# xiaochuanle/MECAT

Measured on AMD Instinct MI355X. Metric: candidate overlaps/sec, higher is better.
Workload: dtype int32

## Files before the change

mecat_amd/csrc/dw_extend2.hip:

```cpp
#include <stdio.h>
#include <stdlib.h>
#include <string.h>

#include <algorithm>
#include <type_traits>

#include "cns_fwd.h"
#include "dw_defs.h"
#include "dw_helpers.h"

#ifndef RCAP
#define RCAP 1024
#endif
#define SEQ_WORDS2 48
constexpr int FULL_BAND_TOL = (int)(0.3 * SEG_BLK), FULL_MAX_D = (int)(.3 * (SEG_BLK + SEG_BLK));
struct StagedLds {
    uint32_t Qp[SEQ_WORDS2][AL_WAVES * 2];
    uint32_t Tp[SEQ_WORDS2][AL_WAVES * 2];
};
#define STAGED_T_BYTES ((int)offsetof(StagedLds, Tp))
typedef __attribute__((address_space(3))) uint16_t lds_u16_t;
typedef __attribute__((address_space(3))) int16_t lds_i16_t;
__device__ __forceinline__ int ring_ld(uint32_t base, uint32_t pos) { return (int)*(lds_i16_t*)(uintptr_t)(base | (pos & (2 * RCAP - 2))); }
__device__ __forceinline__ void ring_st(uint32_t base, uint32_t pos, int x) { *(lds_u16_t*)(uintptr_t)(base | (pos & (2 * RCAP - 2))) = (uint16_t)x; }

__device__ __forceinline__ int sep_word(int rec) { return rec ^ (int)0xE000FFFFu; }

#define BALLOT(p) __builtin_amdgcn_ballot_w64(p)

template <int CTRL> __device__ __forceinline__ int dpp_max_step(int v) {
    return max(v, __builtin_amdgcn_update_dpp((int)0x80000000, v, CTRL, 0xf, 0xf, false));
}
__device__ __forceinline__ int half_max(int v0) {
    int v;
    asm("s_nop 1\n\tv_max_i32_dpp %0, %1, %1 quad_perm:[1,0,3,2] row_mask:0xf bank_mask:0xf" : "=v"(v) : "v"(v0));
    v = dpp_max_step<0x4E>(v);
    v = dpp_max_step<0x141>(v);
    v = dpp_max_step<0x140>(v);
    int r = v, w = v;
    asm("s_nop 1\n\tv_permlane16_swap_b32 %0, %1\n\ts_nop 1" : "+v"(r), "+v"(w));
    return max(r, w);
}
__device__ __forceinline__ int half_min(int v) { return -half_max(-v); }

template <int OFF> __device__ __forceinline__ unsigned long long bits_at(int n) {
    unsigned long long r;
    asm("s_bfm_b64 %0, %1, %2" : "=s"(r) : "s"(n), "n"(OFF));
    return r;
}

typedef uint32_t dw_u32x2 __attribute__((ext_vector_type(2)));
__device__ __forceinline__ unsigned long long pair64(uint32_t lo, uint32_t hi) {
    const dw_u32x2 v = {lo, hi};
    return __builtin_bit_cast(unsigned long long, v);
}
__device__ __forceinline__ uint32_t word_lo(unsigned long long v) { return __builtin_bit_cast(dw_u32x2, v).x; }
__device__ __forceinline__ uint32_t word_hi(unsigned long long v) { return __builtin_bit_cast(dw_u32x2, v).y; }

__device__ __forceinline__ unsigned long long pass_bits(int n) {
    unsigned long long r;
    asm("s_bfm_b64 %0, %1, 0" : "=s"(r) : "s"(n));
    return r;
}

template <int OFF> __device__ __forceinline__ unsigned long long clamped_bits_at(int n) {
    unsigned long long r;
    int c;
    asm("s_min_i32 %1, %2, 32\n\ts_max_i32 %1, %1, 0\n\ts_bfm_b64 %0, %1, %3" : "=s"(r), "=&s"(c) : "s"(n), "n"(OFF) : "scc");
    return r;
}

#define ROWS_ENDED 0xc0000000u
__device__ __forceinline__ unsigned long long snake_step_end(unsigned long long at_lim, unsigned long long amask, int nn,
                                                             unsigned long long& ended, int& rows_more) {
    unsigned long long more;
    int mark;
    asm("s_and_b64 %[more], %[at], %[am]\n\t"
        "s_cbranch_scc0 1f\n\t"
        "v_cmp_eq_u32 vcc, 32, %[nn]\n\t"
        "s_and_b64 vcc, vcc, %[more]\n\t"
        "s_cselect_b64 %[more], 0, %[more]\n\t"
        "s_cselect_b32 %[mark], 0, 0xc0000000\n\t"
        "s_or_b32 %[rm], %[rm], %[mark]\n\t"
        "s_or_b64 %[en], %[en], %[more]\n\t"
        "s_mov_b64 %[more], vcc\n"
        "1:"
        : [more] "=&s"(more), [mark] "=&s"(mark), [en] "+s"(ended), [rm] "+s"(rows_more)
        : [at] "s"(at_lim), [am] "s"(amask), [nn] "v"(nn)
        : "vcc", "scc");
    return more;
}
__device__ __forceinline__ int rows_more_value(int rows_more, bool marked) {
    return marked ? (int)(((unsigned)rows_more + 1u) & ~ROWS_ENDED) - 1 : rows_more;
}

#ifndef DW2_WAVES_PER_SIMD
#define DW2_WAVES_PER_SIMD 8
#endif
#ifndef CNS_FWD_WAVES_PER_SIMD
#define CNS_FWD_WAVES_PER_SIMD 8
#endif
template <bool CNS>
__global__ __launch_bounds__(AL_BLOCK, CNS ? CNS_FWD_WAVES_PER_SIMD : DW2_WAVES_PER_SIMD) void dw_extend2(const uint32_t* __restrict__ rpac, const mhip_offset_t* __restrict__ roffs,
                                                       const uint32_t* __restrict__ qpac, const mhip_offset_t* __restrict__ qoffs,
                                                       const mhip_aln_job* __restrict__ jobs, int n, DirResult* __restrict__ dres,
                                                       DwHandover* __restrict__ hand, unsigned int* __restrict__ hand_count,
                                                       unsigned int* __restrict__ cursor, unsigned long long* __restrict__ counters,
                                                       const CnsFwdArgs ca) {
    struct DwLds {
        uint16_t rings[AL_WAVES * 2][RCAP];
        StagedLds staged;
    };
    static_assert(offsetof(DwLds, staged) % 2048 == 0 && 32 * SEQ_WORDS2 <= 2048 && sizeof(uint32_t) * AL_WAVES * 2 == 32,
                  "a window's byte offset x2 & ~31 and the address of a half's word 0 have no bit in common");
    __shared__ __attribute__((aligned(2 * RCAP))) DwLds lds;
    const int lane = lane_id(), hh = lane >> 5, sl = lane & 31;
    const int half_u = (threadIdx.x >> 6) * 2 + hh;
    const uint32_t rbase = (uint32_t)(uintptr_t)(lds_u16_t*)&lds.rings[half_u][0];
    const uint32_t ubase = (uint32_t)(uintptr_t)(lds_u32_t*)&lds.staged.Qp[0][half_u];
    unsigned int cells = 0, nblocks = 0, nhand = 0;
#ifdef MECAT_DW_STATS
    unsigned long long nrows = 0, nidle = 0, nwide = 0;
    unsigned long long tk_rows = 0, tk_setup = 0, tk_ended = 0, tk_trace = 0, tk_acct = 0, n_outer = 0, n_setup = 0, n_ended = 0, n_pass3 = 0;
    unsigned long long nh[8] = {0, 0, 0, 0, 0, 0, 0, 0};
    unsigned long long q16[6] = {0, 0, 0, 0, 0, 0};
    unsigned long long snake2 = 0;
    unsigned long long n_one = 0, n_one32 = 0;
    const unsigned long long tk_start = wall_clock64();
#define DWS_T(var) const unsigned long long var = wall_clock64()
#define DWS_ADD(acc, a, b) acc += (b) - (a)
#else
#define DWS_T(var)
#define DWS_ADD(acc, a, b)
#endif

    bool need_unit = true, exhausted = false;
    bool setup = true;
    bool inblock = false;
    unsigned int unit = 0;
    SeqView q, t;
    q.pac = qpac; t.pac = rpac; q.off = 0; t.off = 0; q.A = q.B = t.A = t.B = 0; q.comp = t.comp = 0;
    int query_size = 0, target_size = 0, qidx = 0, tidx = 0;
    int Rq = 0, Rt = 0, Rm = 0, Rc = 0, Rb = 0;
    int q_len2 = 0, t_len2 = 0, last_block = 0, band_tol2 = 0, max_d = 0;
    int best_m = -1, mk_l = 0, nslot = 0, aligned = 0, end_x = 0, end_k = 0, end_d = 0, end_mk = 0, d = 0;
    int sepv = sep_word(1);
    int cut = 0;
    unsigned int lin_l = 0;
    unsigned int pb_l = 0;
    unsigned int rlin_l = 0;
    int dlim = 0;
    unsigned int logpos = 0, logend = 0, blk_log0 = 0, blkpos = 0, blkend = 0;
    bool cns_bad = false;
    unsigned long long fl0 = 0, fl1 = 0, fl2 = 0;
    int last_ns = 0;

    while (true) {
#ifdef MECAT_DW_STATS
        n_outer += 1;
        n_setup += BALLOT(setup) ? 1u : 0u;
#endif
        DWS_T(t_a);
        if (BALLOT(setup)) {
            if (setup && need_unit) {
                unsigned int u = 0;
                if (sl == 0) u = atomicAdd(cursor, 1u);
                u = __shfl(u, hh << 5);
                if (u >= 2u * (unsigned)n) { exhausted = true; setup = false; mk_l = 4 * sl; nslot = 0; dlim = 0; }
                else {
                    unit = u;
                    const mhip_aln_job jb = jobs[u >> 1];
                    const int right = u & 1;
                    const int qsize = qoffs[jb.qid_local].size, tsize = roffs[jb.sid_local].size;
                    q.off = qoffs[jb.qid_local].offset; q.comp = jb.chain;
                    t.off = roffs[jb.sid_local].offset; t.comp = 0;
                    const int qs0 = right ? jb.qstart : jb.qstart - 1, step = right ? 1 : -1;
                    if (jb.chain) { q.A = qsize - 1 - qs0; q.B = -step; } else { q.A = qs0; q.B = step; }
                    t.A = right ? jb.sstart : jb.sstart - 1; t.B = step;
                    if (right) { query_size = qsize - jb.qstart; target_size = tsize - jb.sstart; }
                    else { query_size = jb.qstart; target_size = jb.sstart; }
                    if (jb.qstart < 0 || jb.sstart < 0) { query_size = 0; target_size = 0; }
                    qidx = tidx = 0;
                    Rq = Rt = Rm = Rc = Rb = 0;
                    need_unit = false;
                    if (CNS) { logpos = ca.logbase[u]; logend = ca.logbase[u + 1]; blkpos = ca.blockbase[u]; blkend = ca.blockbase[u + 1]; cns_bad = false; }
                }
            }
            if (setup) {
                const int qleft = query_size - qidx, tleft = target_size - tidx;
                int qblk, tblk, band_tol;
                if (CNS) {
                    const int ext = min(qleft, tleft);
                    if (ext > SEG_BLK + 100) { qblk = SEG_BLK; last_block = 0; } else { qblk = max(ext, 0); last_block = 1; }
                    tblk = qblk;
                    if (last_block) {
                        band_tol = (int)(0.3 * qblk);
                        max_d = (int)(2.0 * ca.error_rate * (qblk + qblk));
                    } else { band_tol = FULL_BAND_TOL; max_d = ca.full_max_d; }
                    blk_log0 = logpos;
                    if (logend - logpos < (unsigned)max_d) { cns_bad = true; max_d = 0; }
                } else {
                if (qleft < SEG_BLK + 100 || tleft < SEG_BLK + 100) {
                    qblk = min(qleft, (int)(tleft + tleft * 0.2));
                    tblk = min(tleft, (int)(qleft + qleft * 0.2));
                    last_block = 1;
                    qblk = max(qblk, 0);
                    tblk = max(tblk, 0);
                    band_tol = (int)(0.3 * (qblk > tblk ? qblk : tblk));
                    max_d = (int)(.3 * (qblk + tblk));
                } else { qblk = SEG_BLK; tblk = SEG_BLK; last_block = 0; band_tol = FULL_BAND_TOL; max_d = FULL_MAX_D; }
                }
                static_assert((SEG_BLK + 99) * 6 / 5 <= 16 * (SEQ_WORDS2 - 1), "the longest block and one 16-base window fit the staged words");
                const int trips = BALLOT(max(qblk, tblk) > 512) ? 2 : 1;
#pragma unroll 1
                for (int w = sl, i = 0; i < trips; w += 32, ++i) {
                    lds_u32_t* const sw = (lds_u32_t*)(uintptr_t)(ubase + 32u * (unsigned)w);
                    if (w * 16 < qblk) sw[0] = view_word_le(q, qidx + w * 16);
                    if (w * 16 < tblk) sw[STAGED_T_BYTES / 4] = view_word_le(t, tidx + w * 16);
                }
                if (sl < 3) ring_st(rbase, 2u * sl, sl == 1 ? 0 : -2);
                best_m = -2; mk_l = 4 * sl; nslot = 1; sepv = sep_word(1); cut = 0;
                aligned = 0; end_x = 0; end_k = 0; end_d = 0; d = 0;
                lin_l = 6u + 2u * sl; pb_l = 2u * sl; rlin_l = 2u * sl;
                dlim = max_d; inblock = true;
                q_len2 = 2 * qblk; t_len2 = 2 * tblk; band_tol2 = 2 * band_tol;
                setup = false;
            }
            __builtin_amdgcn_wave_barrier();
        }
        if (!BALLOT(!exhausted)) break;
        const int k_offset = max_d;
        DWS_T(t_b);
        DWS_ADD(tk_setup, t_a, t_b);

        const unsigned long long inmask = BALLOT(inblock);
        bool row_ok;
        unsigned long long ended = 0;
        int NJ = 1;
        auto band_update = [&](const int NJ, const int m0, const int mp, auto both_tag, int& sa, int& sb) __attribute__((always_inline)) {
            constexpr bool BOTH = decltype(both_tag)::value;
            int first, last;
            int pk = 0;
            if (NJ == 1) {
                const unsigned long long q0 = BALLOT(m0 >= best_m - band_tol2);
                if (BOTH) {
                    const unsigned int wa = (unsigned int)q0, wb = (unsigned int)(q0 >> 32);
                    const int fa = __builtin_ctz(wa), fb = __builtin_ctz(wb);
                    sa = 33 - (fa + __builtin_clz(wa));
                    sb = 33 - (fb + __builtin_clz(wb));
                    unsigned long long pkw = (unsigned int)(sa | (fa << 8)) | ((unsigned long long)(unsigned int)(sb | (fb << 8)) << 32);
                    asm("" : "+s"(pkw));
                    pk = (int)(unsigned int)(pkw >> (hh << 5));
                    first = pk >> 8;
                    last = first + (pk & 0xff) - 2;
                } else {
                    const unsigned int m32 = (unsigned int)(q0 >> (hh << 5));
                    int lz;
                    asm("v_ffbl_b32 %0, %1" : "=v"(first) : "v"(m32));
                    asm("v_ffbh_u32 %0, %1" : "=v"(lz) : "v"(m32));
                    last = 31 - lz;
                }
            } else if (NJ == 2) {
                const int thr = best_m - band_tol2;
                const unsigned long long q0 = BALLOT(mp >= thr), q1 = BALLOT(m0 >= thr);
                if (BOTH) {
                    const unsigned long long wa = pair64(word_lo(q0), word_lo(q1)), wb = pair64(word_hi(q0), word_hi(q1));
                    const int fa = __builtin_ctzll(wa), fb = __builtin_ctzll(wb);
                    sa = 65 - (fa + __builtin_clzll(wa));
                    sb = 65 - (fb + __builtin_clzll(wb));
                    unsigned long long pkw = (unsigned int)(sa | (fa << 8)) | ((unsigned long long)(unsigned int)(sb | (fb << 8)) << 32);
                    asm("" : "+s"(pkw));
                    pk = (int)(unsigned int)(pkw >> (hh << 5));
                    first = pk >> 8;
                    last = first + (pk & 0xff) - 2;
                } else {
                    const unsigned int lo32 = (unsigned int)(q0 >> (hh << 5)), hi32 = (unsigned int)(q1 >> (hh << 5));
                    unsigned int fl, fh, ll, lh;
                    asm("v_ffbl_b32 %0, %1" : "=v"(fl) : "v"(lo32));
                    asm("v_ffbl_b32 %0, %1" : "=v"(fh) : "v"(hi32));
                    asm("v_ffbh_u32 %0, %1" : "=v"(ll) : "v"(lo32));
                    asm("v_ffbh_u32 %0, %1" : "=v"(lh) : "v"(hi32));
                    first = (int)min(fl, fh | 32u);
                    last = max((int)(ll ^ 31u), (int)((lh ^ 31u) | 32u));
                }
            } else {
                int lo = 0x7fffffff, hi = -0x7fffffff;
                for (int j = 0; j < NJ; ++j) {
                    const int tt = sl + 32 * j;
                    const bool act = inblock && tt < nslot;
                    const int k2 = mk_l + 128 * j;
                    const int u = act ? 2 * ring_ld(rbase, rlin_l + 64u * (unsigned)j) - k2 : -0x40000000;
                    if (act && u >= best_m - band_tol2) { lo = min(lo, tt); hi = max(hi, tt); }
                }
                first = half_min(lo); last = half_max(hi);
            }
            if (BOTH || inblock) {
                const unsigned int first2 = twice((unsigned)first), step = first2 - 2u;
                pb_l = rlin_l + step;
                nslot = last - first + 2;
                mk_l = mk_l + (int)first2 + (int)step;
                cut = first;
                if (BOTH && NJ <= 2) sepv = sep_word(pk);
                else {
                    int c7;
                    asm("v_min_u16 %0, 0x7f, %1" : "=v"(c7) : "v"(first));
                    sepv = sep_word(nslot | (c7 << 8));
                }
            }
            if (!(BOTH && NJ <= 2)) { sa = __builtin_amdgcn_readlane(nslot, 0); sb = __builtin_amdgcn_readlane(nslot, 32); }
        };
        int last_m0 = 0, last_mp = 0;
        unsigned int row_bytes = 0;
        auto row_passes = [&](const int NJ, const int ns_a, const int ns_b, int& rows_more, auto fast_tag) __attribute__((always_inline)) {
            constexpr int FAST = decltype(fast_tag)::value;

            row_bytes = twice((unsigned)nslot) + 2u;
            last_ns = nslot;
            int mmax = -0x40000000, m0 = -0x40000000, mp = -0x40000000;
            unsigned long long two_m1 = 0, two_m2 = 0;
            if (FAST == 2) {
                const unsigned long long ma = pass_bits(ns_a), mb = pass_bits(ns_b);
                two_m1 = pair64(word_lo(ma), word_lo(mb));
                two_m2 = pair64(word_hi(ma), word_hi(mb));
            }
            int j = 0;
            do {
                const int tt = sl + 32 * j;
                unsigned long long amask;
                if (FAST == 2) {
                    amask = j == 0 ? two_m1 : two_m2;
                } else if (FAST == 1) {
                    amask = bits_at<0>(ns_a) | bits_at<32>(ns_b);
                } else {
                    amask = clamped_bits_at<0>(ns_a - 32 * j) | clamped_bits_at<32>(ns_b - 32 * j);
                }
                const bool act = __builtin_amdgcn_inverse_ballot_w64(amask);
                const int k2 = mk_l + 128 * j;
                const unsigned int rp = pb_l + 64u * (unsigned)j;
                const int vl = ring_ld(rbase, rp), vr = ring_ld(rbase, rp + 2u);
                int x;
                {
                    int v1;
                    asm("v_add_u16 %0, 2, %1" : "=v"(v1) : "v"(vl));
                    asm("v_max_i16 %0, %1, %2" : "=v"(x) : "v"(v1), "v"(vr));
                    if (CNS) {
                        unsigned long long fb;
                        asm("v_cmp_gt_i16_e64 %0, %1, %2" : "=s"(fb) : "v"(v1), "v"(vr));
                        fl0 = j == 0 ? fb : fl0;
                        fl1 = j == 1 ? fb : fl1;
                        fl2 = j == 2 ? fb : fl2;
                    }
                }
                int y = x - k2;
#ifdef MECAT_DW_STATS
                snake2 -= 1;
#endif
                unsigned long long more;
                do {
#ifdef MECAT_DW_STATS
                    snake2 += 1;
#endif
                    int limc;
                    asm("v_min3_i32 %0, %1, %2, 32" : "=v"(limc) : "v"(q_len2 - x), "v"(t_len2 - y));
                    const int m = match16_le2<STAGED_T_BYTES>(ubase, x, y);
                    const int nn = min(m, limc);
                    x += nn; y += nn;
                    more = snake_step_end(BALLOT(nn == limc), amask, nn, ended, rows_more);
                } while (more);
                const int v = act ? x : sepv;
                if (NJ <= 2 || tt <= nslot) ring_st(rbase, lin_l + 64u * (unsigned)j, v);
                mp = m0;
                m0 = v + y;
                mmax = NJ == 1 ? m0 : max(mmax, m0);
            } while (++j < NJ);
            last_m0 = m0; last_mp = mp;
            rlin_l = lin_l;
            __builtin_amdgcn_wave_barrier();
            best_m = half_max(mmax);
        };
#ifdef MECAT_DW_STATS
        auto row_stats = [&](unsigned long long rmask, int ns_a, int ns_b, int NJ) {
            nrows += 1;
            nidle += (rmask == ~0ull) ? 0u : 1u;
            nwide += NJ > 1 ? 1u : 0u;
            n_pass3 += NJ > 2 ? 1u : 0u;
            if (rmask == ~0ull && max(ns_a, ns_b) <= 32) { n_one += 1; n_one32 += max(ns_a, ns_b) == 32 ? 1u : 0u; }
            for (int hq = 0; hq < 2; ++hq) {
                if (!((rmask >> (hq << 5)) & 1ull)) continue;
                const int ns = hq ? ns_b : ns_a;
                nh[ns <= 8 ? 0 : ns <= 16 ? 1 : ns <= 24 ? 2 : ns <= 32 ? 3 : ns <= 48 ? 4 : ns <= 64 ? 5 : ns <= 96 ? 6 : 7] += 1;
                const int p16 = (ns + 15) >> 4;
                q16[p16 <= 4 ? p16 - 1 : p16 <= 6 ? 4 : 5] += 1;
            }
        };
#define DWS_ROW(rmask, a, b, nj) row_stats(rmask, a, b, nj)
#else
#define DWS_ROW(rmask, a, b, nj)
#endif
        auto log_row = [&](const int NJ, auto both_tag) __attribute__((always_inline)) {
            if constexpr (CNS) {
                constexpr bool BOTH = decltype(both_tag)::value;
                if (BOTH || inblock) {
                    const uint32_t lo = hh ? (uint32_t)(fl0 >> 32) : (uint32_t)fl0, hi = NJ >= 2 ? (hh ? (uint32_t)(fl1 >> 32) : (uint32_t)fl1) : 0u;
                    const uint32_t top = NJ >= 3 ? (hh ? (uint32_t)(fl2 >> 32) : (uint32_t)fl2) : 0u;
                    if (NJ > 3) cns_bad = true;
                    ca.rowlog[logpos] = CnsRowRec{lo, hi, (uint32_t)last_ns | ((uint32_t)cut << 8), top};
                    logpos += 1;
                }
            }
        };
        int ns_a = __builtin_amdgcn_readlane(nslot, 0), ns_b = __builtin_amdgcn_readlane(nslot, 32);
        if (inmask == ~0ull) {
            const int rows_left = min(__builtin_amdgcn_readlane(dlim - d, 0), __builtin_amdgcn_readlane(dlim - d, 32));
            const int lim_a = (__builtin_amdgcn_readlane(band_tol2, 0) >> 1) + 1, lim_b = (__builtin_amdgcn_readlane(band_tol2, 32) >> 1) + 1;
            const int one_a = min(lim_a, 32), one_b = min(lim_b, 32);
            const int two_a = min(lim_a, 63), two_b = min(lim_b, 63);
            typedef std::integral_constant<int, 0> fast0;
            typedef std::integral_constant<int, 1> fast1;
            typedef std::integral_constant<int, 2> fast2;
            int rows_more = rows_left - 1;
            while (true) {
                while ((rows_more | (one_a - ns_a) | (one_b - ns_b)) >= 0) {
                    DWS_ROW(~0ull, ns_a, ns_b, 1);
                    const bool full = ((ns_a | ns_b) & 32) != 0;
                    row_passes(1, ns_a, ns_b, rows_more, fast1{});
                    lin_l += row_bytes;
                    if (full) ring_st(rbase, lin_l - 2u * sl - 2u, sepv);
                    band_update(1, last_m0, last_mp, std::true_type{}, ns_a, ns_b);
                    log_row(1, std::true_type{});
                    rows_more -= 1;
                    __builtin_amdgcn_wave_barrier();
                }
                if (ended) break;
                while ((rows_more | (two_a - ns_a) | (two_b - ns_b) | (max(ns_a, ns_b) - 33)) >= 0) {
                    DWS_ROW(~0ull, ns_a, ns_b, 2);
                    NJ = 2;
                    row_passes(2, ns_a, ns_b, rows_more, fast2{});
                    band_update(2, last_m0, last_mp, std::true_type{}, ns_a, ns_b);
                    log_row(2, std::true_type{});
                    lin_l += row_bytes;
                    rows_more -= 1;
                    __builtin_amdgcn_wave_barrier();
                }
                if (ended) break;
                if (rows_more < 0 || ns_a > lim_a || ns_b > lim_b) break;
                const int ns_max = max(ns_a, ns_b);
                if (ns_max < 64) continue;
                NJ = (ns_max + 31) >> 5;
                DWS_ROW(~0ull, ns_a, ns_b, NJ);
                row_passes(NJ, ns_a, ns_b, rows_more, fast0{});
                rows_more -= 1;
                lin_l += row_bytes;
                if ((ns_max & 31) == 0) ring_st(rbase, lin_l - 2u * sl - 2u, sepv);
                band_update(NJ, last_m0, last_mp, std::true_type{}, ns_a, ns_b);
                log_row(NJ, std::true_type{});
                if (ended) break;
                __builtin_amdgcn_wave_barrier();
            }
            d += rows_left - 1 - rows_more_value(rows_more, ended != 0) - (ended ? 1 : 0);
        } else {
            const int slot_lim = (band_tol2 >> 1) + 1;
            int no_count = 0;
            while (true) {
                const unsigned long long rmask = BALLOT(d < dlim) & BALLOT(nslot <= slot_lim);
                if (rmask != inmask) break;
                const int ns_max = max(ns_a, ns_b);
                NJ = (ns_max + 31) >> 5;
                DWS_ROW(rmask, ns_a, ns_b, NJ);
                row_passes(NJ, ns_a, ns_b, no_count, std::integral_constant<int, 0>{});
                lin_l += row_bytes;
                if ((ns_max & 31) == 0) ring_st(rbase, lin_l - 2u * sl - 2u, sepv);
                band_update(NJ, last_m0, last_mp, std::false_type{}, ns_a, ns_b);
                log_row(NJ, std::false_type{});
                if (ended) break;
                d += 1;
                __builtin_amdgcn_wave_barrier();
            }
        }
        DWS_T(t_c);
        DWS_ADD(tk_rows, t_b, t_c);
#ifdef MECAT_DW_STATS
        n_ended += ended ? 1u : 0u;
#endif
        if (ended) {
            const int en = (int)((lin_l - rlin_l) >> 1) - 1, emk_l = (mk_l >> 1) - 2 * cut + 1;
            const int q_len = q_len2 >> 1, t_len = t_len2 >> 1;
            int hkey = 0x7fffffff;
            for (int j = 0; BALLOT(sl + 32 * j < en); ++j) {
                const int k = emk_l + 64 * j, kk = k + k_offset;
                if (sl + 32 * j < en) {
                    const int x = ring_ld(rbase, rlin_l + 64u * (unsigned)j) >> 1;
                    if (x >= q_len || x - k >= t_len) hkey = min(hkey, (kk << 10) | x);
                }
            }
            hkey = half_min(hkey);
            if (inblock && hkey != 0x7fffffff) {
                aligned = 1; end_k = (hkey >> 10) - k_offset; end_x = hkey & 1023; end_d = d;
                end_mk = emk_l - 2 * sl;
                dlim = 0;
            }
            d += 1;
            __builtin_amdgcn_wave_barrier();
        }
        row_ok = d < dlim && nslot <= (band_tol2 >> 1) + 1;
        DWS_T(t_d);
        DWS_ADD(tk_ended, t_c, t_d);

        const bool fin = inblock && !row_ok;

        bool has_aln = fin && aligned;
        bool handover = !CNS && fin && d > 0 && !aligned;
        const int end_y = end_x - end_k;
        const int aln_size = (end_x + end_y + end_d) / 2;
        int cd = end_d, ck = end_k, cx2 = 2 * end_x;
        int acnt2 = 0, found = 0;
        bool tracing = CNS ? (has_aln && !last_block) : has_aln;
        const unsigned int lin_u = lin_l - 2u * sl;
        unsigned int clin = rlin_l - 2u * sl;
        int cmin = end_mk;
        int sepc = ~ring_ld(rbase, lin_u - 2u);
        while (BALLOT(tracing)) {
            if (tracing) {
                const bool up = cd > 0;
                const int sp = ~ring_ld(rbase, clin - 2u);
                const int pcut = (sepc >> 8) & 127, pns = sp & 255;
                const unsigned int plin = clin - 2u - 2u * (unsigned)pns;
                const bool lost = up && (pcut == 127 || lin_u - plin > 2 * RCAP - 128);
                const int pmin = cmin - 2 * pcut + 1;
                const unsigned int ol = (unsigned)(ck - 1 - pmin), olast = 2u * (unsigned)pns - 2u;
                const int rl = ring_ld(rbase, plin + ol), rr = ring_ld(rbase, plin + ol + 2u);
                const int vl = ol <= olast ? rl : -2, vr = ol + 2u <= olast ? rr : -2;
                const int x1 = up ? max(vl + 2, vr) : 0;
                const int sn = cx2 - x1;
                const bool run4 = sn >= 8;
                const bool go = up && !run4 && !lost;
                acnt2 += run4 ? 8 : sn + (up ? 2 : 0);
                cx2 = run4 ? cx2 - 8 : (up ? max(vl, vr) : 0);
                ck = go ? ck + (vl < vr ? 1 : -1) : ck;
                cd -= go ? 1 : 0;
                found = run4 ? 1 : 0;
                clin = plin; cmin = pmin; sepc = sp;
                handover = handover || lost;
                tracing = go;
            }
        }
        const int cx = cx2 >> 1;
        int acnt = acnt2 >> 1;
        int qcnt = end_x - cx, tcnt = end_y - (cx - ck);
        const int trim_ok = has_aln && found && (aln_size - acnt >= 2);
        DWS_T(t_e);
        DWS_ADD(tk_trace, t_d, t_e);

        const int qblk = q_len2 >> 1, tblk = t_len2 >> 1;
        if (CNS && fin) {
            bool done = true;
            if (handover || cns_bad) {
                if (sl == 0) {
                    ca.hand_units[1u + atomicAdd(ca.hand_units, 1u)] = unit;
                    CnsDir D = {0, 0, 0, 0, 0, -1};
                    ca.dres[unit] = D;
                    nhand += 1;
                }
            } else {
                nblocks += (sl == 0) ? 1u : 0u;
                cells += (sl == 0) ? ((lin_l - 6u) >> 1) - (unsigned)d : 0u;
                bool keep = has_aln && (last_block || found);
                const int kept_q = end_x - qcnt, kept_t = end_y - tcnt, kept_cols = aln_size - acnt;
                keep = keep && kept_q != 0;
                if (keep && Rc + kept_cols > ca.dir_cols_cap) { keep = false; if (sl == 0) atomicExch(ca.err_flag, 1); }
                if (keep && blkpos >= blkend) {
                    if (sl == 0) {
                        ca.hand_units[1u + atomicAdd(ca.hand_units, 1u)] = unit;
                        CnsDir D = {0, 0, 0, 0, 0, -1};
                        ca.dres[unit] = D;
                        nhand += 1;
                    }
                } else {
                    if (keep) {
                        if (sl == 0) {
                            CnsBlockRec B = {unit, qidx, tidx, qblk, end_d, end_k, end_mk, end_x, Rc, kept_cols, blk_log0, 0};
                            ca.blocks[blkpos] = B;
                        }
                        blkpos += 1;
                        Rc += kept_cols; Rq += kept_q; Rt += kept_t;
                        if (!last_block) { qidx += kept_q; tidx += kept_t; done = false; }
                    }
                    if (done && sl == 0) { CnsDir D = {Rc, Rq, Rt, 0, 0, 0}; ca.dres[unit] = D; }
                }
            }
            if (done) need_unit = true;
            inblock = false;
            setup = true;
            dlim = 0;
        }
        if (!CNS && fin) {
            bool stop;
            if (handover) {
                if (sl == 0) {
                    DwHandover h;
                    h.unit = unit; h.qidx = qidx; h.tidx = tidx;
                    h.R.qbases = Rq; h.R.tbases = Rt; h.R.matches = Rm; h.R.columns = Rc; h.R.blocks = Rb; h.R.pad = 0;
                    hand[atomicAdd(hand_count, 1u)] = h;
                    nhand += 1;
                }
                need_unit = true;
            } else {
                nblocks += (sl == 0) ? 1u : 0u;
                cells += (sl == 0) ? ((lin_l - 6u) >> 1) - (unsigned)d : 0u;
                Rb += 1;
                stop = !has_aln || !trim_ok;
                if (!stop) {
                    const int full_map = (qblk - end_x <= 20 || tblk - end_y <= 20);
                    const bool last = last_block || !full_map;
                    if (last) { qcnt -= 4; tcnt -= 4; acnt -= 4; }
                    Rc += (end_x + end_y + end_d) / 2 - acnt;
                    Rm += (end_x + end_y - end_d) / 2 - (qcnt + tcnt - acnt);
                    Rq += end_x - qcnt;
                    Rt += end_y - tcnt;
                    if (last) stop = true;
                    else { qidx += end_x - qcnt; tidx += end_y - tcnt; }
                }
                if (stop) {
                    if (sl == 0) { DirResult R = {Rq, Rt, Rm, Rc, Rb, 0}; dres[unit] = R; }
                    need_unit = true;
                }
            }
            inblock = false;
            setup = true;
            dlim = 0;
        }
        DWS_T(t_f);
        DWS_ADD(tk_acct, t_e, t_f);
    }
    unsigned long long c64 = cells, b64 = nblocks, h64 = nhand;
    for (int off = 32; off > 0; off >>= 1) { b64 += __shfl_xor(b64, off); c64 += __shfl_xor(c64, off); h64 += __shfl_xor(h64, off); }
    if (lane == 0) {
        atomicAdd(&counters[3], b64);
        atomicAdd(&counters[4], c64);
        atomicAdd(&counters[8], h64);
#ifdef MECAT_DW_STATS
        atomicAdd(&counters[9], nrows);
        atomicAdd(&counters[10], nidle);
        atomicAdd(&counters[11], nwide);
        atomicAdd(&counters[16], wall_clock64() - tk_start);
        atomicAdd(&counters[17], tk_setup);
        atomicAdd(&counters[18], tk_rows);
        atomicAdd(&counters[19], tk_ended);
        atomicAdd(&counters[20], tk_trace);
        atomicAdd(&counters[21], tk_acct);
        atomicAdd(&counters[22], n_outer);
        atomicAdd(&counters[23], n_setup);
        atomicAdd(&counters[24], n_ended);
        atomicAdd(&counters[25], n_pass3);
        atomicAdd(&counters[26], 1ull);
        atomicAdd(&counters[27], snake2);
        atomicAdd(&counters[28], n_one);
        atomicAdd(&counters[29], n_one32);
        for (int i = 0; i < 8; ++i) atomicAdd(&counters[32 + i], nh[i]);
        for (int i = 0; i < 6; ++i) atomicAdd(&counters[40 + i], q16[i]);
#endif
    }
}

int dw_extend2_launch(mhip_ctx* c, const mhip_volume* ref, const mhip_volume* reads, const void* d_jobs, int n, DirResult* dres,
                      DwHandover* hand, unsigned int* hand_count, unsigned int* cursor) {
    int waves = DW2_WAVES_PER_SIMD * 4;
    if (const char* e = getenv("MECAT_DW_WAVES")) waves = std::max(4, std::min(32, atoi(e)));
    const int grid = std::min(c->num_cus * waves / AL_WAVES, (n + AL_WAVES - 1) / AL_WAVES);
    if (getenv("MECAT_TRACE")) {
        int nb = 0;
        (void)hipOccupancyMaxActiveBlocksPerMultiprocessor(&nb, dw_extend2<false>, AL_BLOCK, 0);
        fprintf(stderr, "[dw trace] occupancy query: %d blocks of %d threads per CU; grid %d; staged words %zu bytes per half\n", nb, AL_BLOCK, grid,
                sizeof(StagedLds) / (AL_WAVES * 2));
    }
    CnsFwdArgs none;
    memset(&none, 0, sizeof(none));
    LAUNCH(c, "dw_extend2", dw_extend2<false>, grid, AL_BLOCK, 0, (const uint32_t*)ref->d_pac, (const mhip_offset_t*)ref->d_offs,
           (const uint32_t*)reads->d_pac, (const mhip_offset_t*)reads->d_offs, (const mhip_aln_job*)d_jobs, n, dres, hand, hand_count,
           cursor, (unsigned long long*)c->d_counters, none);
    return 0;
}

int cns_forward_launch(mhip_ctx* c, const mhip_volume* ref, const mhip_volume* reads, const void* d_jobs, int n, const CnsFwdArgs& args) {
    unsigned int* d_cur;
    if (c->scratch("cnf_cursor", 64, (void**)&d_cur)) return -1;
    HIPCHK(hipMemsetAsync(d_cur, 0, 16, c->stream));
    const int waves = getenv("MECAT_CNS_WAVES") ? std::max(4, std::min(32, atoi(getenv("MECAT_CNS_WAVES")))) : 4 * CNS_FWD_WAVES_PER_SIMD;
    const int grid = std::min(c->num_cus * waves / AL_WAVES, (n + AL_WAVES - 1) / AL_WAVES);
    CnsFwdArgs a = args;
    a.full_max_d = (int)(2.0 * a.error_rate * (SEG_BLK + SEG_BLK));
    LAUNCH(c, "cns_forward", dw_extend2<true>, grid, AL_BLOCK, 0, (const uint32_t*)ref->d_pac, (const mhip_offset_t*)ref->d_offs,
           (const uint32_t*)reads->d_pac, (const mhip_offset_t*)reads->d_offs, (const mhip_aln_job*)d_jobs, n, (DirResult*)nullptr,
           (DwHandover*)nullptr, (unsigned int*)nullptr, d_cur, (unsigned long long*)c->d_counters, a);
    return 0;
}
```

Before: 6.927 million.

## Replace masked ring addressing with relocating linear ring and link words

Ring loads and stores now use absolute LDS addresses without the per-access base-OR and modulo mask, so the inner row loop saves ALU work. When a row would run past the end of the ring, the write pointer is moved back to the origin and a link word records where the previous segment ended, and traceback follows that link. It also folds per-lane counters into one event register, adds relocation and link counters, and moves some block-end state into loop-local variables. The cost is an extra ballot per row and a relocation check, plus more complex traceback that could lose rows if handled wrongly.

```diff
diff --git a/mecat_amd/csrc/dw_extend2.hip b/mecat_amd/csrc/dw_extend2.hip
--- a/mecat_amd/csrc/dw_extend2.hip
+++ b/mecat_amd/csrc/dw_extend2.hip
@@ -19,10 +19,14 @@
     uint32_t Tp[SEQ_WORDS2][AL_WAVES * 2];
 };
 #define STAGED_T_BYTES ((int)offsetof(StagedLds, Tp))
+#define RING_ORG 3
+#define ROW_STORE 128u
 typedef __attribute__((address_space(3))) uint16_t lds_u16_t;
 typedef __attribute__((address_space(3))) int16_t lds_i16_t;
-__device__ __forceinline__ int ring_ld(uint32_t base, uint32_t pos) { return (int)*(lds_i16_t*)(uintptr_t)(base | (pos & (2 * RCAP - 2))); }
-__device__ __forceinline__ void ring_st(uint32_t base, uint32_t pos, int x) { *(lds_u16_t*)(uintptr_t)(base | (pos & (2 * RCAP - 2))) = (uint16_t)x; }
+template <int OFF = 0> __device__ __forceinline__ int ring_ld(uint32_t pos) { return (int)((lds_i16_t*)(uintptr_t)pos)[OFF / 2]; }
+template <int OFF = 0> __device__ __forceinline__ void ring_st(uint32_t pos, int x) { ((lds_u16_t*)(uintptr_t)pos)[OFF / 2] = (uint16_t)x; }
+#define RING_LINK_BITS 11
+static_assert(2 * RCAP == 1 << RING_LINK_BITS, "a ring offset is the low bits of the word at the origin");
 
 __device__ __forceinline__ int sep_word(int rec) { return rec ^ (int)0xE000FFFFu; }
 
@@ -116,9 +120,15 @@
     __shared__ __attribute__((aligned(2 * RCAP))) DwLds lds;
     const int lane = lane_id(), hh = lane >> 5, sl = lane & 31;
     const int half_u = (threadIdx.x >> 6) * 2 + hh;
-    const uint32_t rbase = (uint32_t)(uintptr_t)(lds_u16_t*)&lds.rings[half_u][0];
+    const uint32_t rbase0 = (uint32_t)(uintptr_t)(lds_u16_t*)&lds.rings[half_u][0];
     const uint32_t ubase = (uint32_t)(uintptr_t)(lds_u32_t*)&lds.staged.Qp[0][half_u];
-    unsigned int cells = 0, nblocks = 0, nhand = 0;
+    const uint32_t wrap_l = rbase0 + (2u * RCAP - ROW_STORE - 2u) + 2u * sl;
+#define RING_BASE(p) ((p) & ~(2u * RCAP - 1u))
+#define org_l (wrap_l - (2u * RCAP - ROW_STORE - 2u - 2u * RING_ORG))
+    unsigned int nev = 0;
+    int pass2_k;
+    asm("s_movk_i32 %0, 0xff80" : "=s"(pass2_k));
+    enum { NEV_HAND = 0, NEV_RELOC = 1, NEV_LINK = 2, NEV_BLOCKS = 3, NEV_CELLS = 4 };
 #ifdef MECAT_DW_STATS
     unsigned long long nrows = 0, nidle = 0, nwide = 0;
     unsigned long long tk_rows = 0, tk_setup = 0, tk_ended = 0, tk_trace = 0, tk_acct = 0, n_outer = 0, n_setup = 0, n_ended = 0, n_pass3 = 0;
@@ -143,12 +153,12 @@
     int query_size = 0, target_size = 0, qidx = 0, tidx = 0;
     int Rq = 0, Rt = 0, Rm = 0, Rc = 0, Rb = 0;
     int q_len2 = 0, t_len2 = 0, last_block = 0, band_tol2 = 0, max_d = 0;
-    int best_m = -1, mk_l = 0, nslot = 0, aligned = 0, end_x = 0, end_k = 0, end_d = 0, end_mk = 0, d = 0;
+    int best_m = -1, mk_l = 0, nslot = 0, d = 0;
     int sepv = sep_word(1);
     int cut = 0;
-    unsigned int lin_l = 0;
-    unsigned int pb_l = 0;
-    unsigned int rlin_l = 0;
+    unsigned int lin_l = org_l + 6u;
+    unsigned int pb_l = org_l;
+    unsigned int rlin_l = org_l;
     int dlim = 0;
     unsigned int logpos = 0, logend = 0, blk_log0 = 0, blkpos = 0, blkend = 0;
     bool cns_bad = false;
@@ -218,10 +228,10 @@
                     if (w * 16 < qblk) sw[0] = view_word_le(q, qidx + w * 16);
                     if (w * 16 < tblk) sw[STAGED_T_BYTES / 4] = view_word_le(t, tidx + w * 16);
                 }
-                if (sl < 3) ring_st(rbase, 2u * sl, sl == 1 ? 0 : -2);
+                if (sl < 6) ring_st(org_l - 2u * RING_ORG, sl == 3 || sl == 5 ? -2 : 0);
                 best_m = -2; mk_l = 4 * sl; nslot = 1; sepv = sep_word(1); cut = 0;
-                aligned = 0; end_x = 0; end_k = 0; end_d = 0; d = 0;
-                lin_l = 6u + 2u * sl; pb_l = 2u * sl; rlin_l = 2u * sl;
+                d = 0;
+                lin_l = org_l + 6u; pb_l = org_l; rlin_l = org_l;
                 dlim = max_d; inblock = true;
                 q_len2 = 2 * qblk; t_len2 = 2 * tblk; band_tol2 = 2 * band_tol;
                 setup = false;
@@ -234,6 +244,7 @@
         DWS_ADD(tk_setup, t_a, t_b);
 
         const unsigned long long inmask = BALLOT(inblock);
+        int end_x = 0, end_k = 0, end_d = -1, end_mk = 0;
         bool row_ok;
         unsigned long long ended = 0;
         int NJ = 1;
@@ -289,7 +300,7 @@
                     const int tt = sl + 32 * j;
                     const bool act = inblock && tt < nslot;
                     const int k2 = mk_l + 128 * j;
-                    const int u = act ? 2 * ring_ld(rbase, rlin_l + 64u * (unsigned)j) - k2 : -0x40000000;
+                    const int u = act ? 2 * ring_ld(rlin_l + 64u * (unsigned)j) - k2 : -0x40000000;
                     if (act && u >= best_m - band_tol2) { lo = min(lo, tt); hi = max(hi, tt); }
                 }
                 first = half_min(lo); last = half_max(hi);
@@ -337,7 +348,7 @@
                 const bool act = __builtin_amdgcn_inverse_ballot_w64(amask);
                 const int k2 = mk_l + 128 * j;
                 const unsigned int rp = pb_l + 64u * (unsigned)j;
-                const int vl = ring_ld(rbase, rp), vr = ring_ld(rbase, rp + 2u);
+                const int vl = ring_ld(rp), vr = ring_ld<2>(rp);
                 int x;
                 {
                     int v1;
@@ -351,7 +362,7 @@
                         fl2 = j == 2 ? fb : fl2;
                     }
                 }
-                int y = x - k2;
+                int y = (FAST == 2 && j == 1) ? (x - mk_l) + pass2_k : x - k2;
 #ifdef MECAT_DW_STATS
                 snake2 -= 1;
 #endif
@@ -368,7 +379,7 @@
                     more = snake_step_end(BALLOT(nn == limc), amask, nn, ended, rows_more);
                 } while (more);
                 const int v = act ? x : sepv;
-                if (NJ <= 2 || tt <= nslot) ring_st(rbase, lin_l + 64u * (unsigned)j, v);
+                if (NJ <= 2 || tt <= nslot) ring_st(lin_l + 64u * (unsigned)j, v);
                 mp = m0;
                 m0 = v + y;
                 mmax = NJ == 1 ? m0 : max(mmax, m0);
@@ -409,6 +420,26 @@
                 }
             }
         };
+        auto ring_relocate = [&]() __attribute__((always_inline)) {
+            const unsigned int ext = max(twice((unsigned)nslot), ROW_STORE);
+            const bool need = lin_l + (ext - ROW_STORE) > wrap_l;
+            if (BALLOT(need)) {
+                if (need) {
+                    const uint32_t rbase = RING_BASE(wrap_l), lin_u = lin_l - 2u * sl, off = lin_u - rbase;
+                    lds_u32_t* const org = (lds_u32_t*)(uintptr_t)rbase;
+                    const int behind = ring_ld(lin_u - 2u);
+                    const uint32_t skew = (*org >> RING_LINK_BITS) + ((off - 2u * RING_ORG) >> 1);
+                    if (sl == 0) { *org = (off - 2u) | (skew << RING_LINK_BITS); ring_st<4>(rbase, behind); }
+                    lin_l = org_l;
+                    nev += (inblock && sl == NEV_RELOC) ? 1u : 0u;
+                }
+                __builtin_amdgcn_wave_barrier();
+            }
+        };
+        auto ring_wraps = [&]() __attribute__((always_inline)) {
+            const unsigned long long w = BALLOT(lin_l > wrap_l);
+            return (int)(word_lo(w) | word_hi(w));
+        };
         int ns_a = __builtin_amdgcn_readlane(nslot, 0), ns_b = __builtin_amdgcn_readlane(nslot, 32);
         if (inmask == ~0ull) {
             const int rows_left = min(__builtin_amdgcn_readlane(dlim - d, 0), __builtin_amdgcn_readlane(dlim - d, 32));
@@ -420,19 +451,22 @@
             typedef std::integral_constant<int, 2> fast2;
             int rows_more = rows_left - 1;
             while (true) {
-                while ((rows_more | (one_a - ns_a) | (one_b - ns_b)) >= 0) {
+                ring_relocate();
+                int wraps = 0;
+                while ((rows_more | (one_a - ns_a) | (one_b - ns_b) | wraps) >= 0) {
                     DWS_ROW(~0ull, ns_a, ns_b, 1);
                     const bool full = ((ns_a | ns_b) & 32) != 0;
                     row_passes(1, ns_a, ns_b, rows_more, fast1{});
                     lin_l += row_bytes;
-                    if (full) ring_st(rbase, lin_l - 2u * sl - 2u, sepv);
+                    if (full) ring_st(lin_l - 2u * sl - 2u, sepv);
                     band_update(1, last_m0, last_mp, std::true_type{}, ns_a, ns_b);
                     log_row(1, std::true_type{});
                     rows_more -= 1;
+                    wraps = ring_wraps();
                     __builtin_amdgcn_wave_barrier();
                 }
                 if (ended) break;
-                while ((rows_more | (two_a - ns_a) | (two_b - ns_b) | (max(ns_a, ns_b) - 33)) >= 0) {
+                while ((rows_more | (two_a - ns_a) | (two_b - ns_b) | (max(ns_a, ns_b) - 33) | wraps) >= 0) {
                     DWS_ROW(~0ull, ns_a, ns_b, 2);
                     NJ = 2;
                     row_passes(2, ns_a, ns_b, rows_more, fast2{});
@@ -440,18 +474,19 @@
                     log_row(2, std::true_type{});
                     lin_l += row_bytes;
                     rows_more -= 1;
+                    wraps = ring_wraps();
                     __builtin_amdgcn_wave_barrier();
                 }
                 if (ended) break;
                 if (rows_more < 0 || ns_a > lim_a || ns_b > lim_b) break;
                 const int ns_max = max(ns_a, ns_b);
-                if (ns_max < 64) continue;
+                if (ns_max < 64 || wraps < 0) continue;
                 NJ = (ns_max + 31) >> 5;
                 DWS_ROW(~0ull, ns_a, ns_b, NJ);
                 row_passes(NJ, ns_a, ns_b, rows_more, fast0{});
                 rows_more -= 1;
                 lin_l += row_bytes;
-                if ((ns_max & 31) == 0) ring_st(rbase, lin_l - 2u * sl - 2u, sepv);
+                if ((ns_max & 31) == 0) ring_st(lin_l - 2u * sl - 2u, sepv);
                 band_update(NJ, last_m0, last_mp, std::true_type{}, ns_a, ns_b);
                 log_row(NJ, std::true_type{});
                 if (ended) break;
@@ -464,12 +499,13 @@
             while (true) {
                 const unsigned long long rmask = BALLOT(d < dlim) & BALLOT(nslot <= slot_lim);
                 if (rmask != inmask) break;
+                ring_relocate();
                 const int ns_max = max(ns_a, ns_b);
                 NJ = (ns_max + 31) >> 5;
                 DWS_ROW(rmask, ns_a, ns_b, NJ);
                 row_passes(NJ, ns_a, ns_b, no_count, std::integral_constant<int, 0>{});
                 lin_l += row_bytes;
-                if ((ns_max & 31) == 0) ring_st(rbase, lin_l - 2u * sl - 2u, sepv);
+                if ((ns_max & 31) == 0) ring_st(lin_l - 2u * sl - 2u, sepv);
                 band_update(NJ, last_m0, last_mp, std::false_type{}, ns_a, ns_b);
                 log_row(NJ, std::false_type{});
                 if (ended) break;
@@ -489,13 +525,13 @@
             for (int j = 0; BALLOT(sl + 32 * j < en); ++j) {
                 const int k = emk_l + 64 * j, kk = k + k_offset;
                 if (sl + 32 * j < en) {
-                    const int x = ring_ld(rbase, rlin_l + 64u * (unsigned)j) >> 1;
+                    const int x = ring_ld(rlin_l + 64u * (unsigned)j) >> 1;
                     if (x >= q_len || x - k >= t_len) hkey = min(hkey, (kk << 10) | x);
                 }
             }
             hkey = half_min(hkey);
             if (inblock && hkey != 0x7fffffff) {
-                aligned = 1; end_k = (hkey >> 10) - k_offset; end_x = hkey & 1023; end_d = d;
+                end_k = (hkey >> 10) - k_offset; end_x = hkey & 1023; end_d = d;
                 end_mk = emk_l - 2 * sl;
                 dlim = 0;
             }
@@ -508,8 +544,8 @@
 
         const bool fin = inblock && !row_ok;
 
-        bool has_aln = fin && aligned;
-        bool handover = !CNS && fin && d > 0 && !aligned;
+        bool has_aln = fin && end_d >= 0;
+        bool handover = !CNS && fin && d > 0 && end_d < 0;
         const int end_y = end_x - end_k;
         const int aln_size = (end_x + end_y + end_d) / 2;
         int cd = end_d, ck = end_k, cx2 = 2 * end_x;
@@ -518,17 +554,23 @@
         const unsigned int lin_u = lin_l - 2u * sl;
         unsigned int clin = rlin_l - 2u * sl;
         int cmin = end_mk;
-        int sepc = ~ring_ld(rbase, lin_u - 2u);
+        int sepc = ~ring_ld(lin_u - 2u);
+        bool crossed = false;
         while (BALLOT(tracing)) {
             if (tracing) {
                 const bool up = cd > 0;
-                const int sp = ~ring_ld(rbase, clin - 2u);
+                const int sp = ~ring_ld(clin - 2u);
                 const int pcut = (sepc >> 8) & 127, pns = sp & 255;
-                const unsigned int plin = clin - 2u - 2u * (unsigned)pns;
-                const bool lost = up && (pcut == 127 || lin_u - plin > 2 * RCAP - 128);
+                const bool cross = (clin & (2u * RCAP - 1u)) == 2u * RING_ORG;
+                const uint32_t link = *(lds_u32_t*)(uintptr_t)RING_BASE(clin) & (2u * RCAP - 1u);
+                const unsigned int plin = (cross ? RING_BASE(clin) | link : clin - 2u) - 2u * (unsigned)pns;
+                const bool over = crossed || cross;
+                const bool lost = up && (pcut == 127 || (over && (int)(plin - lin_u) < (int)ROW_STORE));
+                nev += (up && cross && sl == NEV_LINK) ? 1u : 0u;
+                crossed = over;
                 const int pmin = cmin - 2 * pcut + 1;
                 const unsigned int ol = (unsigned)(ck - 1 - pmin), olast = 2u * (unsigned)pns - 2u;
-                const int rl = ring_ld(rbase, plin + ol), rr = ring_ld(rbase, plin + ol + 2u);
+                const int rl = ring_ld(plin + ol), rr = ring_ld<2>(plin + ol);
                 const int vl = ol <= olast ? rl : -2, vr = ol + 2u <= olast ? rr : -2;
                 const int x1 = up ? max(vl + 2, vr) : 0;
                 const int sn = cx2 - x1;
@@ -559,11 +601,11 @@
                     ca.hand_units[1u + atomicAdd(ca.hand_units, 1u)] = unit;
                     CnsDir D = {0, 0, 0, 0, 0, -1};
                     ca.dres[unit] = D;
-                    nhand += 1;
+                    nev += 1;
                 }
             } else {
-                nblocks += (sl == 0) ? 1u : 0u;
-                cells += (sl == 0) ? ((lin_l - 6u) >> 1) - (unsigned)d : 0u;
+                nev += (sl == NEV_BLOCKS) ? 1u : 0u;
+                nev += (sl == NEV_CELLS) ? ((lin_l - org_l - 6u) >> 1) + (*(lds_u32_t*)(uintptr_t)RING_BASE(wrap_l) >> RING_LINK_BITS) - (unsigned)d : 0u;
                 bool keep = has_aln && (last_block || found);
                 const int kept_q = end_x - qcnt, kept_t = end_y - tcnt, kept_cols = aln_size - acnt;
                 keep = keep && kept_q != 0;
@@ -573,7 +615,7 @@
                         ca.hand_units[1u + atomicAdd(ca.hand_units, 1u)] = unit;
                         CnsDir D = {0, 0, 0, 0, 0, -1};
                         ca.dres[unit] = D;
-                        nhand += 1;
+                        nev += 1;
                     }
                 } else {
                     if (keep) {
@@ -601,12 +643,12 @@
                     h.unit = unit; h.qidx = qidx; h.tidx = tidx;
                     h.R.qbases = Rq; h.R.tbases = Rt; h.R.matches = Rm; h.R.columns = Rc; h.R.blocks = Rb; h.R.pad = 0;
                     hand[atomicAdd(hand_count, 1u)] = h;
-                    nhand += 1;
+                    nev += 1;
                 }
                 need_unit = true;
             } else {
-                nblocks += (sl == 0) ? 1u : 0u;
-                cells += (sl == 0) ? ((lin_l - 6u) >> 1) - (unsigned)d : 0u;
+                nev += (sl == NEV_BLOCKS) ? 1u : 0u;
+                nev += (sl == NEV_CELLS) ? ((lin_l - org_l - 6u) >> 1) + (*(lds_u32_t*)(uintptr_t)RING_BASE(wrap_l) >> RING_LINK_BITS) - (unsigned)d : 0u;
                 Rb += 1;
                 stop = !has_aln || !trim_ok;
                 if (!stop) {
@@ -632,12 +674,15 @@
         DWS_T(t_f);
         DWS_ADD(tk_acct, t_e, t_f);
     }
-    unsigned long long c64 = cells, b64 = nblocks, h64 = nhand;
-    for (int off = 32; off > 0; off >>= 1) { b64 += __shfl_xor(b64, off); c64 += __shfl_xor(c64, off); h64 += __shfl_xor(h64, off); }
+    unsigned long long c64 = sl == NEV_CELLS ? nev : 0u, b64 = sl == NEV_BLOCKS ? nev : 0u;
+    unsigned long long h64 = sl == NEV_HAND ? nev : 0u, r64 = sl == NEV_RELOC ? nev : 0u, l64 = sl == NEV_LINK ? nev : 0u;
+    for (int off = 32; off > 0; off >>= 1) { b64 += __shfl_xor(b64, off); c64 += __shfl_xor(c64, off); h64 += __shfl_xor(h64, off); r64 += __shfl_xor(r64, off); l64 += __shfl_xor(l64, off); }
     if (lane == 0) {
         atomicAdd(&counters[3], b64);
         atomicAdd(&counters[4], c64);
         atomicAdd(&counters[8], h64);
+        atomicAdd(&counters[30], r64);
+        atomicAdd(&counters[31], l64);
 #ifdef MECAT_DW_STATS
         atomicAdd(&counters[9], nrows);
         atomicAdd(&counters[10], nidle);
```

Result: faster. 7.036 million, median of 6 (+1.6%).
